# minfenli/refnerf-pl

Hardware: AMD Instinct MI355X
Metric: ray-samples/s (4096 rays x 128 samples x 2 levels, Ref-NeRF Blender, eval forward) (higher is better)
Workload: dtype f16x2; 1 GPU; blender_refnerf.gin, 4096 rays x 128 samples, 2-level, Model.__call__ eval forward with compute_extras + full ray_history; rays_per_gpu=4096, total_rays=4096, samples_per_level=128, parallelism=ray-tile dp1, n_ranks_seen=1, hip_graph_replay=False

## Files before the change

### refnerf-pl_amd/csrc/refnerf_level_bf16.h

```cpp
#pragma once
#include <type_traits>

#include "refnerf_level_common.h"

namespace rn {

typedef short v2s __attribute__((ext_vector_type(2)));

struct MmBf16 {
  typedef __bf16 t;
  typedef t v8 __attribute__((ext_vector_type(8)));
  typedef t v2 __attribute__((ext_vector_type(2)));
  static __device__ __forceinline__ v16f mfma(v8 a, v8 b, v16f c) { return __builtin_amdgcn_mfma_f32_32x32x16_bf16(a, b, c, 0, 0, 0); }
};
struct MmF16 {
  typedef _Float16 t;
  typedef t v8 __attribute__((ext_vector_type(8)));
  typedef t v2 __attribute__((ext_vector_type(2)));
  static __device__ __forceinline__ v16f mfma(v8 a, v8 b, v16f c) { return __builtin_amdgcn_mfma_f32_32x32x16_f16(a, b, c, 0, 0, 0); }
};
template <typename MM>
__device__ __forceinline__ unsigned cvt_pk_mm(float lo, float hi) {
  typename MM::v2 r = __builtin_convertvector((v2f){lo, hi}, typename MM::v2);
  return __builtin_bit_cast(unsigned, r);
// ... 428 lines not shown
  if (KIND == SQ_BN) return 2 * (j / 4) + (j & 1);
  if (KIND == SQ_SC) return 2 * (j / 3) + ((j % 3) == 1 ? 1 : 0);
  return 4 * (j / 6) + ((j % 6) < 4 ? (j % 6) : (j % 6) - 4);
}
template <int KIND> constexpr bool sq_lo(int j) { return KIND == SQ_BN ? (j & 3) >= 2 : (KIND == SQ_SC ? (j % 3) == 2 : (j % 6) >= 4); }
template <int KIND> constexpr int sq_tile(int j) { return KIND == SQ_SC ? 0 : (KIND == SQ_BN ? (j & 1) : ((j % 6) & 1)); }
template <int KIND> constexpr int sq_release(int j) {
  if (KIND == SQ_BN) return (j & 3) >= 2 ? 2 * (j / 4) + ((j & 3) - 2) : -1;
  if (KIND == SQ_SC) return (j % 3) == 1 ? 2 * (j / 3) + 1 : ((j % 3) == 2 ? 2 * (j / 3) : -1);
  const int jj = j % 6, sl = j / 6;
  return jj == 2 ? 4 * sl + 2 : (jj == 3 ? 4 * sl + 3 : (jj == 4 ? 4 * sl : (jj == 5 ? 4 * sl + 1 : -1)));
}
template <int KIND, bool PRE, typename Hook = NoHook>
__device__ __forceinline__ void sq_chunk(Pipe &p, sq_v8 (&fr)[SQ_NF], const v4uu (&in)[16], SqAcc &acc, SqAcc &nacc, Hook &&hook = Hook(), int adv = BF_CHUNK_BYTES) {
  constexpr int NM = sq_nm<KIND>(), NP = sq_np<KIND>();
  constexpr int RDV = NM / 2 - 1;
  const char *w = p.wbuf + p.cur_off;
  const char *cur = w + 1024 + p.lane * 16;
  const char *nxt = p.wbuf + p.nxt_off + 1024 + p.lane * 16;
  sq_v8 xb[2];
  if (KIND == SQ_X) { xb[0] = lds_frag<MmF16>(p.xps); xb[1] = lds_frag<MmF16>(p.xps + (BT / 2) * 16); }
  __builtin_amdgcn_sched_barrier(0);
#pragma unroll
  for (int j = 0; j < NM; ++j) {
    const int sl = sq_step<KIND>(j);
    sq_v8 b;
    if (KIND == SQ_X) b = xb[sq_lo<KIND>(j) ? 1 : 0];
    else b = __builtin_bit_cast(sq_v8, in[2 * ((KIND == SQ_B ? 4 : 0) + sl) + (sq_lo<KIND>(j) ? 1 : 0)]);
    if (sq_tile<KIND>(j)) acc.t1 = __builtin_amdgcn_mfma_f32_16x16x32_f16(fr[sq_piece<KIND>(j) % SQ_NF], b, acc.t1, 0, 0, 0);
    else acc.t0 = __builtin_amdgcn_mfma_f32_16x16x32_f16(fr[sq_piece<KIND>(j) % SQ_NF], b, acc.t0, 0, 0, 0);
    const int rel = sq_release<KIND>(j);
    if (rel >= 0) {
      const int q = rel + SQ_NF;
      fr[rel % SQ_NF] = (q < NP) ? lds_frag<MmF16>(cur + q * 1024) : lds_frag<MmF16>(nxt + (q - NP) * 1024);
    }
    hook(j);
    if (KIND == SQ_X) {
      if ((j % 6) == 3 && sl + 1 < 3) xb[0] = lds_frag<MmF16>(p.xps + (sl + 1) * (4 * BT * 16));
      if ((j % 6) == 5 && sl + 1 < 3) xb[1] = lds_frag<MmF16>(p.xps + (sl + 1) * (4 * BT * 16) + (BT / 2) * 16);
    }
    if (j == RDV) {
      RN_RENDEZVOUS(p);
      issue_chunk<true>(p, p.fil_off, 0);
      if (PRE) {
        const v4f *bp = reinterpret_cast<const v4f *>(p.wbuf + p.nxt_off + (p.lane >> 4) * 16);
        nacc.t0 = bp[0];
        nacc.t1 = bp[4];
      }
    }
    if (j == RDV + 4) issue_chunk<true>(p, p.fil_off, 1);
    if (j == RDV + 8) issue_chunk<true>(p, p.fil_off, 2, adv);
    __builtin_amdgcn_sched_barrier(0);
  }
  ring_rotate(p);
}
__device__ __forceinline__ void sq_epi_piece(const SqAcc &a, int q, v4uu &oh, v4uu &ol) {
  const float y0 = q == 0 ? a.t0[0] : (q == 1 ? a.t0[2] : (q == 2 ? a.t1[0] : a.t1[2]));
  const float y1 = q == 0 ? a.t0[1] : (q == 1 ? a.t0[3] : (q == 2 ? a.t1[1] : a.t1[3]));
  const float x0 = (y0 < 0.0f) ? 0.0f : y0, x1 = (y1 < 0.0f) ? 0.0f : y1;
  unsigned hi, lo;
  split_pair_f16(x0, x1, hi, lo);
  oh[q] = hi;
  ol[q] = lo;
}
template <bool LAYER0>
__device__ __forceinline__ void sq_layer(Pipe &p, sq_v8 (&fr)[SQ_NF], SqAcc (&accs)[2], bool skip, const v4uu (&in)[16], v4uu (&out)[16]) {
#pragma unroll
  for (int ob = 0; ob < 8; ++ob) {
    SqAcc &acc = accs[(ob + 1) & 1];
    SqAcc &prev = accs[ob & 1];
    auto hook = [&](int j) {
      if (ob == 0 || j >= 8 || (j & 1)) return;
      sq_epi_piece(prev, j >> 1, out[2 * ob - 2], out[2 * ob - 1]);
    };
    if constexpr (LAYER0) sq_chunk<SQ_XR, true>(p, fr, in, acc, prev, hook);
    else {
      sq_chunk<SQ_A, false>(p, fr, in, acc, prev, hook);
      sq_chunk<SQ_B, true>(p, fr, in, acc, prev);
      if (skip) sq_chunk<SQ_X, true>(p, fr, in, acc, prev);
    }
  }
#pragma unroll
  for (int q = 0; q < 4; ++q) sq_epi_piece(accs[0], q, out[14], out[15]);
  __builtin_amdgcn_sched_barrier(0);
}
__device__ __forceinline__ void sq_load_ipe_frags(const Pipe &p, v4uu (&in)[16]) {
#pragma unroll
  for (int s = 0; s < 3; ++s) {
    in[2 * s] = __builtin_bit_cast(v4uu, lds_frag<MmF16>(p.xps + s * (4 * BT * 16)));
    in[2 * s + 1] = __builtin_bit_cast(v4uu, lds_frag<MmF16>(p.xps + s * (4 * BT * 16) + (BT / 2) * 16));
  }
}
__device__ __forceinline__ void sq_bias_now(const Pipe &p, SqAcc &acc) {
  const v4f *bp = reinterpret_cast<const v4f *>(p.wbuf + p.cur_off + (p.lane >> 4) * 16);
  acc.t0 = bp[0];
  acc.t1 = bp[4];
}

template <typename MM, int KIND0, int REAL0>
__device__ __forceinline__ void dir_layer(Pipe &p, typename MM::v8 (&a)[AF], int second, const v4uu (&in)[16], const v4uu (&bn)[8], v4uu (&out)[16], int adv6 = BF_CHUNK_BYTES) {
#pragma unroll
  for (int ob = 0; ob < 8; ++ob) {
    v16f acc;
    bf_chunk<MM, KIND0, REAL0, true, true>(p, a, in, bn, acc, NoHook(), ob == 6 ? adv6 : BF_CHUNK_BYTES);
    if constexpr (KIND0 == BF_REG) {
      if (second == 2) bf_chunk<MM, BF_BNLDS, BF_DIR_REAL_KS, false, true>(p, a, in, bn, acc);
    }
    pack_acc<MM, true>(acc, out[2 * ob], out[2 * ob + 1]);
    __builtin_amdgcn_sched_barrier(0);
  }
}

template <bool RINGPS = false>
__device__ __forceinline__ void level_fwd_split(const LevelArgs &A) {
  typedef MmF16 MM;
  constexpr int PSM = RINGPS ? BF_PS_RING - 1 : 0;
  typedef typename MM::v8 v8mm;
  typedef typename MM::t mm_t;
  extern __shared__ __attribute__((aligned(16))) float smem[];
  const refnerf_level_cfg &cfg = A.cfg;
  const int N = cfg.n_samples;
  const int tid = threadIdx.x, lane = tid & 63;
  const int wave = __builtin_amdgcn_readfirstlane(tid >> 6);
  const int rpw = A.rpw;
  const int ray0 = blockIdx.x * rpw;
  const int n_tot = rpw * N;
  const int n_pass = (n_tot + BT - 1) / BT;

  char *WB = reinterpret_cast<char *>(smem);
  char *Xb = WB + BF_RING_BYTES;
  float *HD = reinterpret_cast<float *>(Xb + BF_X_BYTES);
  float *TD = HD + HD_ROWS * BT;
  float *XP = TD + rpw * (N + 1);
  float *PS = XP + rpw * (N + 1);
  float *PX = PS + (RINGPS ? BF_PS_RING : n_tot) * NPS_EVAL;
  float *NRM = PX + 3 * BT;
  const float *RY = NRM + 8;

  const int h = lane >> 5, n = lane & 31;
  const int col = wave * 32 + n;

  Pipe p;
  pipe_stream_init(p, A.packed, n_pass * SPPACKED.chunks_per_pass, wave, lane);
  p.wbuf = WB;
  p.xp = Xb + (h * BT + col) * 16;
  p.xps = Xb + ((lane >> 4) * BT + wave * 16 + (lane & 15)) * 16;
  p.cur_off = 0; p.nxt_off = BF_CHUNK_BYTES; p.fil_off = 2 * BF_CHUNK_BYTES;
  p.lane = lane; p.wave = wave; p.h = h;
  p.t_vm = 0; p.t_bar = 0;
  RN_STAMPW(A, 0);
#ifdef REFNERF_PROF_WAITS
  if (A.prof && blockIdx.x == (gridDim.x >> 1) && lane == 0) A.prof[wave * 32 + 22] = (long long)__builtin_amdgcn_s_memrealtime();
#endif
  issue_chunk<true>(p, p.cur_off);
  issue_chunk<true>(p, p.nxt_off);

  resample_phase<BF_NW, true>(A, reinterpret_cast<float *>(Xb), TD, NRM, ray0, wave, lane);
#pragma clang loop unroll(disable)
  for (int rl = wave; rl < rpw; rl += BF_NW) {
    const int ray = ray0 + rl;
    if (ray >= A.R) break;
    float *RYw = NRM + 8 + rl * 12;
    if (lane < 10) {
      const float val = lane < 3 ? A.rays.d_origins[(size_t)ray * 3 + lane]
                      : lane < 6 ? A.rays.d_directions[(size_t)ray * 3 + lane - 3]
                      : lane < 9 ? A.rays.d_viewdirs[(size_t)ray * 3 + lane - 6] : A.rays.d_radii[ray];
      RYw[lane] = val;
      const float dx = __shfl(val, 3, 64), dy = __shfl(val, 4, 64), dz = __shfl(val, 5, 64);
      if (lane == 0) NRM[rl] = sqrtf((dx * dx + dy * dy) + dz * dz);
    }
  }
  RN_STAMPW(A, 1);
  asm volatile("s_waitcnt vmcnt(0)" ::: "memory");
  __syncthreads();
  RN_STAMPW(A, 2);

  if (wave >= BF_NW / 2) __builtin_amdgcn_s_setprio(1);
  v4uu R0[16], R1[16];
  sq_v8 ar[SQ_NF];
#pragma unroll
  for (int d = 0; d < SQ_NF; ++d) ar[d] = lds_frag<MM>(WB + 1024 + lane * 16 + d * 1024);

  for (int pass0 = 0; pass0 < n_tot; pass0 += BT) {
    int lane_v = lane;
    asm volatile("" : "+v"(lane_v));
    p.lane_off = (unsigned)(wave * 3072 + lane_v * 16);
    auto locate = [&](int &g, int &rl, bool &valid) {
      int col_l = col, pass_l = pass0;
      asm volatile("" : "+v"(col_l), "+s"(pass_l));
      g = pass_l + col_l;
      rl = g / N;
      valid = (g < n_tot) && (ray0 + rl < A.R);
    };
    auto pass_epilogue = [&]() {
      if constexpr (RINGPS) {
        __syncthreads();
        const int end = (pass0 + BT < n_tot) ? pass0 + BT : n_tot;
        int td_o = (int)(TD - smem), xp_o = (int)(XP - smem), ps_o = (int)(PS - smem), nrm_o = (int)(NRM - smem), lane_e = lane, pass_e = pass0;
        int ntot_e = n_tot, ray0_e = ray0, wave_e = wave;
        asm volatile("" : "+s"(td_o), "+s"(xp_o), "+s"(ps_o), "+s"(nrm_o), "+v"(lane_e), "+s"(pass_e), "+s"(ntot_e), "+s"(ray0_e), "+s"(wave_e));
        composite_phase<BF_NW, false, NPS_EVAL, PSM>(A, smem + td_o, smem + xp_o, smem + ps_o, ntot_e, ray0_e, wave_e, lane_e, nullptr, smem + nrm_o,
                                                     pass_e / N, end / N);
      }
    };
    {
      const int g0 = pass0 + wave * 32;
      if (g0 >= n_tot || ray0 + g0 / N >= A.R) { idle_pass<true>(p); pass_epilogue(); continue; }
    }
    auto load_heads = [&](SampleHeads &sh, int &g, bool &valid) {
      int rl;
      locate(g, rl, valid);
      int ci = col, ro = (valid ? rl : 0) * 12;
      asm volatile("" : "+v"(ci), "+v"(ro));
      float v[3], gp[3], raw_dif[3], raw_tint[3];
#pragma unroll
      for (int i = 0; i < 3; ++i) {
        v[i] = RY[ro + 6 + i];
        gp[i] = HD[(1 + i) * BT + ci];
        raw_dif[i] = HD[(5 + i) * BT + ci];
        raw_tint[i] = HD[(8 + i) * BT + ci];
      }
      sample_heads<false>(cfg, HD[0 * BT + ci], gp, HD[4 * BT + ci], raw_dif, raw_tint, v, sh);
    };

    v4uu bn0[4];
    auto heads = [&](auto RUN, v4uu (&bn)[8]) {
      constexpr int run = decltype(RUN)::value;
      SqAcc ha[2];
      sq_bias_now(p, ha[1]);
#pragma unroll
      for (int ob = 0; ob < 5; ++ob) {
        SqAcc &acc = ha[(ob + 1) & 1];
        if (ob < 4) {
          sq_chunk<SQ_BN, true>(p, ar, R1, acc, ha[ob & 1], NoHook(), (run == 0 && ob == 2) ? SP_ADV_REWIND : BF_CHUNK_BYTES);
#pragma unroll
          for (int e = 0; e < 4; ++e) {
            const unsigned pk = e == 0 ? pk_f16(acc.t0[0], acc.t0[1]) : (e == 1 ? pk_f16(acc.t0[2], acc.t0[3])
                              : (e == 2 ? pk_f16(acc.t1[0], acc.t1[1]) : pk_f16(acc.t1[2], acc.t1[3])));
            if (run == 0) bn0[ob][e] = pk;
            else {
              const v2uu r = __builtin_amdgcn_permlane16_swap(bn0[ob][e], pk, false, false);
              bn[2 * ob][e] = r[0];
              bn[2 * ob + 1][e] = r[1];
            }
          }
        } else {
          sq_chunk<SQ_SC, false>(p, ar, R1, acc, ha[ob & 1]);
          const int bq = lane_v >> 4;
          int csl = wave * 32 + 16 * run + (lane_v & 15) + 4 * bq * BT;
          asm volatile("" : "+v"(csl));
#pragma unroll
          for (int i = 0; i < 4; ++i)
            if (4 * bq + i < HD_ROWS) HD[i * BT + csl] = acc.t0[i];
        }
      }
      wave_sync();
    };
    typedef std::integral_constant<int, 0> Run0;
    typedef std::integral_constant<int, 1> Run1;

#pragma unroll 1
    for (int phase = 0; phase < 2; ++phase) {
#pragma unroll
      for (int e = 0; e < 16; ++e) { R0[e] = (v4uu){0, 0, 0, 0}; R1[e] = (v4uu){0, 0, 0, 0}; }
      {
      const int i16 = lane_v & 15, part = lane_v >> 4;
      const int hb = part >> 1, qq = part & 1;
      const int cs = wave * 32 + 16 * phase + i16;
      const int gs = pass0 + cs;
      const int rls = gs / N, sis = gs - rls * N;
      const bool vs = (gs < n_tot) && (ray0 + rls < A.R);
      float o[3], d[3];
      const float *ry = RY + (vs ? rls : 0) * 12;
#pragma unroll
      for (int i = 0; i < 3; ++i) { o[i] = ry[i]; d[i] = ry[3 + i]; }
      const float radius = ry[9];
      const float *td = TD + (vs ? rls : 0) * (N + 1);
      const float t0 = td[vs ? sis : 0], t1 = td[vs ? sis + 1 : 1];
      float lm[3], lv[3];
      cast_sample(o, d, radius, t0, t1, cfg.ray_shape, lm, lv);
      if (cfg.disable_integration) { lv[0] = 0.0f; lv[1] = 0.0f; lv[2] = 0.0f; }
      char *xw = Xb + (wave * 16 + i16) * 16;
      RN_STAMPW(A, 17);
      float sc = qq ? 256.0f : 1.0f, sc2 = qq ? 65536.0f : 1.0f;
      char *xq = xw + (6 * hb + 3 * qq) * BT * 16;
#pragma clang loop unroll(disable)
      for (int dp = 0; dp < 4; ++dp) {
        const float sc_odd = sc * 2.0f, sc2_odd = sc2 * 4.0f;
#pragma unroll
        for (int a = 0; a < 3; ++a) {
          float f[2];
#pragma unroll
          for (int u = 0; u < 2; ++u) {
            const int k6 = 2 * a + u, odd = k6 / 3, b3 = k6 - 3 * odd;
            f[u] = ipe_feature_split_sc(lm[b3], lv[b3], odd ? sc_odd : sc, odd ? sc2_odd : sc2, hb);
          }
          unsigned whi, wlo;
          split_pair_f16(f[0], f[1], whi, wlo);
          const int t = 3 * dp + a;
          char *dst = xq + (t >> 2) * BT * 16 + (t & 3) * 4;
          *reinterpret_cast<unsigned *>(dst) = whi;
          *reinterpret_cast<unsigned *>(dst + (BT / 2) * 16) = wlo;
        }
        sc *= 4.0f;
        sc2 *= 16.0f;
      }
      }
      RN_STAMPW(A, 18);
      wave_sync();
      RN_STAMPW(A, 3 + phase * 4);
      if (phase == 0) {
#pragma unroll
        for (int d = AF; d < SQ_NF; ++d) ar[d] = lds_frag<MM>(p.wbuf + p.cur_off + 1024 + lane_v * 16 + d * 1024);
      }
      SqAcc accs[2];
      sq_bias_now(p, accs[1]);
      sq_load_ipe_frags(p, R1);
      sq_layer<true>(p, ar, accs, false, R1, R0);
#pragma unroll
      for (int e = 0; e < 6; ++e) R1[e] = (v4uu){0, 0, 0, 0};
      RN_STAMPW(A, 4 + phase * 4);
#pragma unroll 1
      for (int it = 0; it < 4; ++it) {
        sq_layer<false>(p, ar, accs, it == 2, R0, R1);
        if (it < 3) sq_layer<false>(p, ar, accs, false, R1, R0);
      }
      RN_STAMPW(A, 5 + phase * 4);
      if (phase == 0) {
        v4uu none[8];
        heads(Run0(), none);
        RN_STAMPW(A, 6);
      }
    }
    v4uu bn[8];
    heads(Run1(), bn);
    RN_STAMPW(A, 10);
#pragma unroll
    for (int e = 0; e < 16; ++e) { R0[e] = (v4uu){0, 0, 0, 0}; R1[e] = (v4uu){0, 0, 0, 0}; }
    {
    const int h4 = RINGPS ? (fresh_lane() >> 5) : h;
    char *xs = Xb + col * 16;
    {
      SampleHeads sh;
      int g4; bool valid4;
      load_heads(sh, g4, valid4);
      if (valid4 && h4 == 0) heads_store<NPS_EVAL, PSM>(sh, PS, PX, g4, RINGPS ? wave * 32 + (fresh_lane() & 31) : col);
      float ide[40];
#pragma unroll
      for (int q = 36; q < 40; ++q) ide[q] = 0.0f;
      if (cfg.dir_enc == REFNERF_DIRENC_POSENC) posenc_eval<false, true>(sh.refd[0], sh.refd[1], sh.refd[2], h4, [&](int q, float val) { ide[q] = val; });
      else ide_eval<false>(sh.refd[0], sh.refd[1], sh.refd[2], sh.rough, h4, [&](int q, float val) { ide[q] = val; });
      if (h4 == 0) ide[36] = sh.dot;
#pragma unroll
      for (int q = 0; q < 5; ++q) {
        v8mm pk;
#pragma unroll
        for (int e = 0; e < 8; ++e) pk[e] = (mm_t)ide[q * 8 + e];
        *reinterpret_cast<v8mm *>(xs + (5 * h4 + q) * BT * 16) = pk;
      }
    }
    wave_sync();
    RN_STAMPW(A, 11);
    v8mm (&ad)[AF] = reinterpret_cast<v8mm (&)[AF]>(ar);
    dir_layer<MM, BF_BNLDS, BF_DIR_REAL_KS>(p, ad, 0, R0, bn, R0);
    RN_STAMPW(A, 12);
#pragma unroll 1
    for (int it = 0; it < 4; ++it) {
      dir_layer<MM, BF_REG, 0>(p, ad, (it == 2) ? 2 : 0, R0, bn, R1, it == 3 ? SP_ADV_WRAP : BF_CHUNK_BYTES);
      if (it < 3) dir_layer<MM, BF_REG, 0>(p, ad, 0, R1, bn, R0);
    }
    RN_STAMPW(A, 13);
    v16f acc;
    bf_chunk<MM, BF_REG, 0, true, true>(p, ad, R1, bn, acc);
    float raw_rgb[3];
    const int lane6 = RINGPS ? fresh_lane() : lane;
    const int n6 = RINGPS ? (lane6 & 31) : n, h6 = RINGPS ? (lane6 >> 5) : h;
#pragma unroll
    for (int i = 0; i < 3; ++i) raw_rgb[i] = __shfl(acc[i], n6, 64);
    int g_w, rl_w; bool valid;
    locate(g_w, rl_w, valid);
    int lane_w = lane6, pass_w = pass0;
    asm volatile("" : "+v"(lane_w), "+s"(pass_w));
    if (valid) {
      int ci = RINGPS ? wave * 32 + n6 : col, pr = ps_row<PSM>(g_w) * NPS_EVAL;
      asm volatile("" : "+v"(ci), "+v"(pr));
      float tint[3], raw_dif[3];
#pragma unroll
      for (int i = 0; i < 3; ++i) { tint[i] = PS[pr + PS_TINT + i]; raw_dif[i] = HD[(5 + i) * BT + ci]; }
      int half = h6;
      asm volatile("" : "+v"(half));
      colour_store_halves<NPS_EVAL, PSM, true>(A, half, tint, raw_dif, raw_rgb, PS, g_w);
    }
    wave_sync();
    history_flush<NPS_EVAL, PSM>(A, PS, PX, n_tot, pass_w + wave * 32, wave * 32, (size_t)ray0 * N + pass_w + wave * 32, lane_w);
    RN_STAMPW(A, 14);
    }
    __builtin_amdgcn_wave_barrier();
    pass_epilogue();
  }
  asm volatile("s_waitcnt vmcnt(0)" ::: "memory");
  __syncthreads();
  RN_STAMPW(A, 15);
#ifdef REFNERF_PROF_WAITS
  if (A.prof && blockIdx.x == (gridDim.x >> 1) && lane == 0) {
    A.prof[wave * 32 + 20] = p.t_vm; A.prof[wave * 32 + 21] = p.t_bar;
    A.prof[wave * 32 + 23] = (long long)__builtin_amdgcn_s_memrealtime();
  }
#endif
  if constexpr (!RINGPS) composite_phase<BF_NW, false, NPS_EVAL>(A, TD, XP, PS, n_tot, ray0, wave, lane, reinterpret_cast<float *>(WB), NRM);
  RN_STAMPW(A, 16);
}

#ifndef REFNERF_SECONDARY_TU
__global__ __launch_bounds__(BF_NTHREADS) void level_fwd_f16x2(const LevelArgs A) { level_fwd_split<false>(A); }
__global__ __launch_bounds__(BF_NTHREADS) void level_fwd_f16x2_ring(const LevelArgs A) { level_fwd_split<true>(A); }
#endif

__device__ __forceinline__ int ipe_col_of_kprime(int kp) { return kp; }

}
```

### refnerf-pl_amd/csrc/refnerf_level_common.h

```cpp
#pragma once
#include <hip/hip_runtime.h>

#include "refnerf_hip.h"
#include "refnerf_device_math.h"
#include "refnerf_layout.h"

namespace rn {

typedef float v16f __attribute__((ext_vector_type(16)));
typedef float v4f __attribute__((ext_vector_type(4)));
typedef unsigned int v4u __attribute__((ext_vector_type(4)));

constexpr int NTHREADS = 256;

typedef __bf16 v8bf __attribute__((ext_vector_type(8)));
typedef unsigned v4uu __attribute__((ext_vector_type(4)));
typedef __bf16 v2bf __attribute__((ext_vector_type(2)));
typedef float v2f __attribute__((ext_vector_type(2)));
__device__ __forceinline__ unsigned cvt_pk_bf16(float lo, float hi) {
  v2bf r = __builtin_convertvector((v2f){lo, hi}, v2bf);
  return __builtin_bit_cast(unsigned, r);
}

constexpr int HD_ROWS = 12;
// ... 43 lines not shown
#pragma unroll
  for (int o = 32; o > 0; o >>= 1) v += __shfl_xor(v, o, 64);
  return v;
}
__device__ __forceinline__ float wave_max(float v) {
#pragma unroll
  for (int o = 32; o > 0; o >>= 1) v = fmaxf(v, __shfl_xor(v, o, 64));
  return v;
}
constexpr int WSUM_PITCH = 65;
template <int K>
__device__ __forceinline__ void wave_sum_many(float (&v)[K], float *scr, int lane) {
#pragma unroll
  for (int k = 0; k < K; ++k) scr[k * WSUM_PITCH + lane] = v[k];
  __builtin_amdgcn_fence(__ATOMIC_SEQ_CST, "wavefront");
  __builtin_amdgcn_wave_barrier();
  float s = 0.0f;
  if (lane < K) {
    const float *col = scr + lane * WSUM_PITCH;
#pragma clang loop unroll(disable)
    for (int j = 0; j < 64; j += 4) s += (col[j] + col[j + 1]) + (col[j + 2] + col[j + 3]);
  }
#pragma unroll
  for (int k = 0; k < K; ++k) v[k] = __shfl(s, k, 64);
  __builtin_amdgcn_fence(__ATOMIC_SEQ_CST, "wavefront");
  __builtin_amdgcn_wave_barrier();
}

__device__ __forceinline__ float lane_value(float x, int l) {
  return __builtin_bit_cast(float, __builtin_amdgcn_readlane(__builtin_bit_cast(int, x), l));
}

__device__ __forceinline__ double wave_scan_incl(double v, int lane) {
#pragma unroll
  for (int o = 1; o < 64; o <<= 1) {
    double t = __shfl_up(v, o, 64);
    if (lane >= o) v += t;
  }
  return v;
}

__device__ __forceinline__ float cdf_interp(float u, float xp0, float xp1, float fp0, float fp1) {
  float q = (u - xp0) / (xp1 - xp0);
  if (q != q) q = 0.0f;
  float off = clip01(q);
  return fp0 + off * (fp1 - fp0);
}

__device__ __forceinline__ void centres_to_sdist(const float *c, int N, float smin, float smax, float *sd, int lane) {
  __builtin_amdgcn_fence(__ATOMIC_SEQ_CST, "wavefront");
  __builtin_amdgcn_wave_barrier();
  #pragma clang loop unroll(disable)
  for (int k = lane; k <= N; k += 64) {
    float v;
    if (k == 0) v = fmaxf(smin, 2.0f * c[0] - (c[1] + c[0]) / 2.0f);
    else if (k == N) v = fminf(smax, 2.0f * c[N - 1] - (c[N - 1] + c[N - 2]) / 2.0f);
    else v = (c[k] + c[k - 1]) / 2.0f;
    sd[k] = v;
  }
  __builtin_amdgcn_fence(__ATOMIC_SEQ_CST, "wavefront");
  __builtin_amdgcn_wave_barrier();
}

template <bool EXACT = true>
__device__ __forceinline__ void build_cdf_wave(float *lg, float *cw, int M, int lane) {
  float mx = -INFINITY;
  #pragma clang loop unroll(disable)
  for (int i = lane; i < M; i += 64) mx = fmaxf(mx, lg[i]);
  mx = wave_max(mx);
  #pragma clang loop unroll(disable)
  for (int i = lane; i < M; i += 64) lg[i] = rn_det_expf(lg[i] - mx);
  __builtin_amdgcn_fence(__ATOMIC_SEQ_CST, "wavefront");
  __builtin_amdgcn_wave_barrier();
  float sum = 0.0f;
  if (EXACT) {
    #pragma clang loop unroll(disable)
    for (int i0 = 0; i0 < M; i0 += 64) {
      const float x = (i0 + lane < M) ? lg[i0 + lane] : 0.0f;
#pragma unroll
      for (int l = 0; l < 64; ++l) sum += lane_value(x, l);
    }
  } else {
    #pragma clang loop unroll(disable)
    for (int i = lane; i < M; i += 64) sum += lg[i];
    sum = wave_sum(sum);
  }
  #pragma clang loop unroll(disable)
  for (int i = lane; i < M; i += 64) lg[i] = lg[i] / sum;
  __builtin_amdgcn_fence(__ATOMIC_SEQ_CST, "wavefront");
  __builtin_amdgcn_wave_barrier();
  if (EXACT) {
    double acc = 0.0;
    #pragma clang loop unroll(disable)
    for (int i0 = 0; i0 < M; i0 += 64) {
      const float x = (i0 + lane < M) ? lg[i0 + lane] : 0.0f;
      float mine = 0.0f;
#pragma unroll
      for (int l = 0; l < 64; ++l) {
        acc += (double)lane_value(x, l);
        mine = (lane == l) ? (float)acc : mine;
      }
      if (i0 + lane < M - 1) cw[i0 + lane + 1] = fminf(1.0f, mine);
    }
    if (lane == 0) { cw[0] = 0.0f; cw[M] = 1.0f; }
  } else {
    const int Cn = (M + 63) / 64, i0 = lane * Cn;
    double loc = 0.0;
    #pragma clang loop unroll(disable)
    for (int q = 0; q < Cn; ++q) if (i0 + q < M - 1) loc += (double)lg[i0 + q];
    double run = wave_scan_incl(loc, lane) - loc;
    #pragma clang loop unroll(disable)
    for (int q = 0; q < Cn; ++q) if (i0 + q < M - 1) { run += (double)lg[i0 + q]; cw[i0 + q + 1] = fminf(1.0f, (float)run); }
    if (lane == 0) { cw[0] = 0.0f; cw[M] = 1.0f; }
  }
  __builtin_amdgcn_fence(__ATOMIC_SEQ_CST, "wavefront");
  __builtin_amdgcn_wave_barrier();
}

__device__ __forceinline__ void invert_cdf_wave(const float *t_in, const float *cw, float *c, int M, int N, float smin, float smax,
                                                float *sd, int32_t *bin_idx_g, int lane) {
  #pragma clang loop unroll(disable)
  for (int k = lane; k < N; k += 64) {
    float u = linspace_u(k, N);
    int lo = 0, hi = M;
    #pragma clang loop unroll(disable)
    while (hi - lo > 1) {
      int mid = (lo + hi) >> 1;
      if (u >= cw[mid]) lo = mid; else hi = mid;
    }
    c[k] = cdf_interp(u, cw[lo], cw[lo + 1], t_in[lo], t_in[lo + 1]);
    if (bin_idx_g) bin_idx_g[k] = lo;
  }
  centres_to_sdist(c, N, smin, smax, sd, lane);
}

template <bool EXACT = true>
__device__ __forceinline__ void sample_intervals_wave(const float *t_in, float *lg, float *cw, float *c, int M, int N,
                                      float smin, float smax, float *sd, int32_t *bin_idx_g, int lane) {
  build_cdf_wave<EXACT>(lg, cw, M, lane);
  invert_cdf_wave(t_in, cw, c, M, N, smin, smax, sd, bin_idx_g, lane);
}

__device__ __forceinline__ int fresh_lane() {
  int z = 0;
  asm volatile("" : "+v"(z));
  return (int)__builtin_amdgcn_mbcnt_hi(~0u, __builtin_amdgcn_mbcnt_lo(~0u, (unsigned)z));
}

__device__ __forceinline__ void st3(float *base, size_t idx, float a, float b, float c) {
  if (base) { base[idx * 3 + 0] = a; base[idx * 3 + 1] = b; base[idx * 3 + 2] = c; }
}


template <int NW = 4, bool EXACT = true>
__device__ __forceinline__ void resample_phase(const LevelArgs &A, float *scratch, float *TD, float *NRM, int ray0, int wave, int lane) {
  const refnerf_level_cfg &cfg = A.cfg;
  const int N = cfg.n_samples, M = cfg.n_in, rpw = A.rpw;
  const int Mp = (M + 4) & ~3, Np = (N + 3) & ~3;
  float *scr = scratch + wave * (3 * Mp + Np);
  float *t_in = scr, *lg = scr + Mp, *cw = scr + 2 * Mp, *c = scr + 3 * Mp;
  #pragma clang loop unroll(disable)
  for (int rl = wave; rl < rpw; rl += NW) {
    int ray = ray0 + rl;
    if (ray >= A.R) break;
    float *sd = TD + rl * (N + 1);
    int32_t *bin_g = A.out.d_bin_idx ? A.out.d_bin_idx + (size_t)ray * N : nullptr;
    if (A.sdist_in == nullptr) {
      t_in[0] = cfg.s_near; t_in[1] = cfg.s_far;
      cw[0] = 0.0f; cw[1] = 1.0f;
      wave_sync();
    } else {
      const float *tg = A.sdist_in + (size_t)ray * (M + 1);
      const float *wg = A.weights_in + (size_t)ray * M;
      #pragma clang loop unroll(disable)
      for (int i = lane; i <= M; i += 64) t_in[i] = tg[i];
      wave_sync();
      RN_STAMP_P0(A, 24);
      #pragma clang loop unroll(disable)
      for (int i = lane; i < M; i += 64)
        lg[i] = (t_in[i + 1] > t_in[i]) ? cfg.anneal * rn_det_logf(wg[i] + cfg.resample_padding) : -INFINITY;
      wave_sync();
      RN_STAMP_P0(A, 25);
      build_cdf_wave<EXACT>(lg, cw, M, lane);
    }
    RN_STAMP_P0(A, 26);
    invert_cdf_wave(t_in, cw, c, M, N, cfg.s_near, cfg.s_far, sd, bin_g, lane);
    RN_STAMP_P0(A, 27);
    float nearv = A.rays.d_near[ray], farv = A.rays.d_far[ray];
    if (!EXACT) {
      float *RY = NRM + 8 + rl * 12;
      if (lane < 10) {
        const float val = lane < 3 ? A.rays.d_origins[(size_t)ray * 3 + lane]
                        : lane < 6 ? A.rays.d_directions[(size_t)ray * 3 + lane - 3]
                        : lane < 9 ? A.rays.d_viewdirs[(size_t)ray * 3 + lane - 6] : A.rays.d_radii[ray];
        RY[lane] = val;
        const float dx = __shfl(val, 3, 64), dy = __shfl(val, 4, 64), dz = __shfl(val, 5, 64);
        if (lane == 0) NRM[rl] = sqrtf((dx * dx + dy * dy) + dz * dz);
      }
    }
    RN_STAMP_P0(A, 28);
    #pragma clang loop unroll(disable)
    for (int k = lane; k <= N; k += 64) {
      float s = sd[k];
      if (A.out.d_sdist) A.out.d_sdist[(size_t)ray * (N + 1) + k] = s;
      sd[k] = s_to_t(s, nearv, farv, A.cfg.raydist);
    }
  }
}

struct SampleHeads {
  float density, rough, dot;
  float tint[3], raw_dif[3], npred[3], gp[3], refd[3];
  float normals[3] = {0.0f, 0.0f, 0.0f};
};
template <bool FAST = false>
__device__ __forceinline__ void sample_heads(const refnerf_level_cfg &cfg, float raw_density, const float gp[3],
                                             float raw_rough, const float raw_dif[3], const float raw_tint[3],
                                             const float v[3], SampleHeads &s) {
#pragma unroll
  for (int i = 0; i < 3; ++i) { s.gp[i] = gp[i]; s.raw_dif[i] = raw_dif[i]; s.tint[i] = sigmoid_m<FAST>(raw_tint[i]); }
  float n2 = fmaxf((gp[0] * gp[0] + gp[1] * gp[1]) + gp[2] * gp[2], EPS32);
  float nrm = sqrtf(n2);
#pragma unroll
  for (int i = 0; i < 3; ++i) s.npred[i] = -m_div<FAST>(gp[i], nrm);
  s.density = softplus_m<FAST>(raw_density + cfg.density_bias);
  s.rough = softplus_m<FAST>(raw_rough + cfg.roughness_bias);
  float w3[3] = {-v[0], -v[1], -v[2]};
  float dot = (s.npred[0] * w3[0] + s.npred[1] * w3[1]) + s.npred[2] * w3[2];
#pragma unroll
  for (int i = 0; i < 3; ++i) s.refd[i] = (2.0f * dot) * s.npred[i] - w3[i];
  s.dot = (s.npred[0] * v[0] + s.npred[1] * v[1]) + s.npred[2] * v[2];
}

template <int PSM>
__device__ __forceinline__ int ps_row(int g) { return PSM ? (g & PSM) : g; }

template <bool FAST = false, int NP = NPS_TRAIN, int PSM = 0, bool FAST_SRGB = FAST, bool PAD_HERE = false>
__device__ __forceinline__ void colour_store(const LevelArgs &A, const SampleHeads &s, const float raw_rgb[3],
                                             float *PS, float *PX, int n_tot, int g_sample, int gcol) {
  const int g = ps_row<PSM>(g_sample);
  const refnerf_level_cfg &cfg = A.cfg;
  float spec_lin[3], dif_lin[3], rgb[3], dif[3], spc[3];
#pragma unroll
  for (int i = 0; i < 3; ++i) {
    float sg = sigmoid_m<FAST>(cfg.rgb_premultiplier * raw_rgb[i] + cfg.rgb_bias);
    dif_lin[i] = sigmoid_m<FAST>(s.raw_dif[i] - LOG3_F);
    spec_lin[i] = s.tint[i] * sg;
    rgb[i] = spec_lin[i] + dif_lin[i];
  }
  if (cfg.srgb_mapping) {
    if (cfg.srgb_mapping_normalization) {
      float norm = fmaxf(fmaxf(fmaxf(rgb[0], rgb[1]), rgb[2]), 1.0f);
#pragma unroll
      for (int i = 0; i < 3; ++i) rgb[i] = m_div<FAST>(rgb[i], norm);
    }
#pragma unroll
    for (int i = 0; i < 3; ++i) {
      rgb[i] = clip01(linear_to_srgb<FAST_SRGB>(rgb[i]));
      dif[i] = clip01(linear_to_srgb<FAST_SRGB>(dif_lin[i]));
      spc[i] = clip01(linear_to_srgb<FAST_SRGB>(spec_lin[i]));
    }
  } else {
#pragma unroll
    for (int i = 0; i < 3; ++i) { dif[i] = dif_lin[i]; spc[i] = spec_lin[i]; }
  }
  float pad = cfg.rgb_padding;
  if (PAD_HERE) asm volatile("" : "+s"(pad));
  const float pad_scale = (float)(1.0 + 2.0 * (double)pad);
#pragma unroll
  for (int i = 0; i < 3; ++i) rgb[i] = rgb[i] * pad_scale - pad;
  PS[g * NP + PS_DENSITY] = s.density;
  PS[g * NP + PS_ROUGH] = s.rough;
#pragma unroll
  for (int i = 0; i < 3; ++i) {
    PS[g * NP + PS_RGB + i] = rgb[i];
    PS[g * NP + PS_DIF + i] = dif[i];
    PS[g * NP + PS_SPC + i] = spc[i];
    PS[g * NP + PS_NPRED + i] = s.npred[i];
    PS[g * NP + PS_TINT + i] = s.tint[i];
    if (NP > PS_NORMALS) PS[g * NP + PS_NORMALS + i] = s.normals[i];
    PX[gcol * 3 + i] = s.gp[i];
  }
}

template <int NP, int PSM>
__device__ __forceinline__ void heads_store(const SampleHeads &s, float *PS, float *PX, int g_sample, int gcol) {
  const int g = ps_row<PSM>(g_sample);
  PS[g * NP + PS_DENSITY] = s.density;
  PS[g * NP + PS_ROUGH] = s.rough;
#pragma unroll
  for (int i = 0; i < 3; ++i) {
    PS[g * NP + PS_NPRED + i] = s.npred[i];
    PS[g * NP + PS_TINT + i] = s.tint[i];
    PX[gcol * 3 + i] = s.gp[i];
  }
}
template <int NP, int PSM, bool PAD_HERE>
__device__ __forceinline__ void colour_store_halves(const LevelArgs &A, int half, const float tint[3], const float raw_dif[3],
                                                    const float raw_rgb[3], float *PS, int g_sample) {
  const int g = ps_row<PSM>(g_sample);
  const refnerf_level_cfg &cfg = A.cfg;
  float own[3], rgb[3];
#pragma unroll
  for (int i = 0; i < 3; ++i) {
    const float sg = sigmoid_m<false>(half ? raw_dif[i] - LOG3_F : cfg.rgb_premultiplier * raw_rgb[i] + cfg.rgb_bias);
    own[i] = half ? sg : tint[i] * sg;
  }
#pragma unroll
  for (int i = 0; i < 3; ++i) rgb[i] = own[i] + __shfl_xor(own[i], 32, 64);
  if (cfg.srgb_mapping) {
    if (cfg.srgb_mapping_normalization) {
      float norm = fmaxf(fmaxf(fmaxf(rgb[0], rgb[1]), rgb[2]), 1.0f);
#pragma unroll
      for (int i = 0; i < 3; ++i) rgb[i] = m_div<false>(rgb[i], norm);
    }
#pragma unroll
    for (int i = 0; i < 3; ++i) {
      rgb[i] = clip01(linear_to_srgb<true>(rgb[i]));
      own[i] = clip01(linear_to_srgb<true>(own[i]));
    }
  }
  float pad = cfg.rgb_padding;
  if (PAD_HERE) asm volatile("" : "+s"(pad));
  const float pad_scale = (float)(1.0 + 2.0 * (double)pad);
  const int own_slot = half ? PS_DIF : PS_SPC;
#pragma unroll
  for (int i = 0; i < 3; ++i) {
    PS[g * NP + own_slot + i] = own[i];
    if (!half) PS[g * NP + PS_RGB + i] = rgb[i] * pad_scale - pad;
  }
}

__device__ __forceinline__ void hist_store(float *p, float v) { __builtin_nontemporal_store(v, p); }
constexpr int AUX_NT = 2;

template <int NP = NPS_TRAIN, int PSM = 0>
__device__ __forceinline__ void history_flush(const LevelArgs &A, const float *PS, const float *PX, int n_tot, int gw0, int gcol0,
                                              size_t gs0, int lane) {
  const size_t total = (size_t)A.R * A.cfg.n_samples;
  auto vec3 = [&](float *dst, int slot) {
    if (!dst) return;
#pragma unroll
    for (int it = 0; it < 2; ++it) {
      const int f = lane + 64 * it;
      const int smp = f / 3, c = f - 3 * smp;
      if (f < 96 && gw0 + smp < n_tot && gs0 + smp < total) hist_store(dst + gs0 * 3 + f, PS[ps_row<PSM>(gw0 + smp) * NP + slot + c]);
    }
  };
  auto scal = [&](float *dst, int slot) {
    if (dst && lane < 32 && gw0 + lane < n_tot && gs0 + lane < total) hist_store(dst + gs0 + lane, PS[ps_row<PSM>(gw0 + lane) * NP + slot]);
  };
  scal(A.out.d_density, PS_DENSITY);
  scal(A.out.d_roughness, PS_ROUGH);
  vec3(A.out.d_rgb, PS_RGB);
  vec3(A.out.d_diffuse, PS_DIF);
  vec3(A.out.d_specular, PS_SPC);
  vec3(A.out.d_normals_pred, PS_NPRED);
  if (A.out.d_grad_pred) {
#pragma unroll
    for (int it = 0; it < 2; ++it) {
      const int f = lane + 64 * it;
      const int smp = f / 3;
      if (f < 96 && gw0 + smp < n_tot && gs0 + smp < total) hist_store(A.out.d_grad_pred + gs0 * 3 + f, PX[gcol0 * 3 + f]);
    }
  }
  vec3(A.out.d_tint, PS_TINT);
  if (NP > PS_NORMALS && A.cfg.training) vec3(A.out.d_normals, PS_NORMALS);
}

template <typename T>
__device__ __forceinline__ T *late_ptr(T *p) {
  asm volatile("" : "+s"(p));
  return p;
}

__device__ __forceinline__ void pct_store(double *soa, double *aos, int R, int ray, int p, double v) {
  if (soa) soa[(size_t)p * R + ray] = v;
  else aos[(size_t)ray * 3 + p] = v;
}

template <int NW = 4, bool FAST = false, int NP = NPS_TRAIN, int PSM = 0>
__device__ __forceinline__ void composite_phase(const LevelArgs &A, const float *TD, float *XP, float *PS, int n_tot,
                                                int ray0, int wave, int lane, float *wscr, const float *NRM,
                                                int rl_begin = 0, int rl_end = -1) {
  const refnerf_level_cfg &cfg = A.cfg;
  const int N = cfg.n_samples, rpw = A.rpw;
  if (rl_end < 0) rl_end = rpw;
  #pragma clang loop unroll(disable)
  for (int rl = rl_begin + wave; rl < rl_end; rl += NW) {
    const int ray = ray0 + rl;
    if (ray >= A.R) break;
    const float *td = TD + rl * (N + 1);
    const int base = rl * N;
    const int C = (N + 63) / 64;
    const int i0 = lane * C;
    float norm;
    if (FAST) norm = NRM[rl];
    else {
      float dx = A.rays.d_directions[(size_t)ray * 3], dy = A.rays.d_directions[(size_t)ray * 3 + 1], dz = A.rays.d_directions[(size_t)ray * 3 + 2];
      norm = sqrtf((dx * dx + dy * dy) + dz * dz);
    }
    auto wref = [&](int i) -> float & { return PS[ps_row<PSM>(base + i) * NP + PS_DENSITY]; };
    auto rec = [&](int i, int slot) { return PS[ps_row<PSM>(base + i) * NP + slot]; };
    double local = 0.0;
    #pragma clang loop unroll(disable)
    for (int q = 0; q < C; ++q) {
      int i = i0 + q;
      if (i < N) {
        float dd = wref(i) * ((td[i + 1] - td[i]) * norm);
        if (!(cfg.opaque_background && i == N - 1)) local += (double)dd;
      }
    }
    double incl = wave_scan_incl(local, lane);
    double cum = incl - local;
    float acc = 0, s_rgb[3] = {0, 0, 0}, s_dif[3] = {0, 0, 0}, s_spc[3] = {0, 0, 0}, s_np[3] = {0, 0, 0}, s_tn[3] = {0, 0, 0};
    float s_nm[3] = {0, 0, 0};
    float s_dist = 0, s_rgh = 0, s_logd = 0;
    double wlocal = 0.0;
    #pragma clang loop unroll(disable)
    for (int q = 0; q < C; ++q) {
      int i = i0 + q;
      if (i < N) {
        float dd = wref(i) * ((td[i + 1] - td[i]) * norm);
        if (cfg.opaque_background && i == N - 1) dd = INFINITY;
        float alpha = 1.0f - m_exp<FAST>(-dd);
        float trans = m_exp<FAST>(-(float)cum);
        float w = alpha * trans;
        cum += (double)dd;
        wref(i) = w;
        wlocal += (double)w;
        if (A.out.d_weights) A.out.d_weights[(size_t)ray * N + i] = w;
        acc += w;
        float tmid = 0.5f * (td[i] + td[i + 1]);
        s_dist += w * tmid;
        s_logd += w * m_log<FAST>(tmid);
        s_rgh += w * rec(i, PS_ROUGH);
#pragma unroll
        for (int c = 0; c < 3; ++c) {
          s_rgb[c] += w * rec(i, PS_RGB + c);
          s_dif[c] += w * rec(i, PS_DIF + c);
          s_spc[c] += w * rec(i, PS_SPC + c);
          s_np[c] += w * rec(i, PS_NPRED + c);
          s_tn[c] += w * rec(i, PS_TINT + c);
          if (NP > PS_NORMALS) s_nm[c] += w * rec(i, PS_NORMALS + c);
        }
      }
    }
    {
      float red[22] = {acc, s_dist, s_logd, s_rgh, s_rgb[0], s_rgb[1], s_rgb[2], s_dif[0], s_dif[1], s_dif[2],
                       s_spc[0], s_spc[1], s_spc[2], s_np[0], s_np[1], s_np[2], s_tn[0], s_tn[1], s_tn[2],
                       s_nm[0], s_nm[1], s_nm[2]};
      if constexpr (PSM != 0) {
#pragma unroll
        for (int k = 0; k < 22; ++k) red[k] = wave_sum(red[k]);
      } else wave_sum_many<22>(red, wscr + wave * (22 * WSUM_PITCH), lane);
      acc = red[0]; s_dist = red[1]; s_logd = red[2]; s_rgh = red[3];
#pragma unroll
      for (int c = 0; c < 3; ++c) {
        s_rgb[c] = red[4 + c]; s_dif[c] = red[7 + c]; s_spc[c] = red[10 + c];
        s_np[c] = red[13 + c]; s_tn[c] = red[16 + c]; s_nm[c] = red[19 + c];
      }
    }
    const float bg_w = fmaxf(0.0f, 1.0f - acc);
    float rgb[3], dif[3], spc[3];
#pragma unroll
    for (int c = 0; c < 3; ++c) {
      rgb[c] = s_rgb[c] + bg_w * cfg.bg_rgb; dif[c] = s_dif[c] + bg_w * cfg.bg_rgb; spc[c] = s_spc[c] + bg_w * cfg.bg_rgb;
    }
    const int mode = cfg.render_srgb_mode;
    if (mode != REFNERF_SRGB_NONE) {
      if (mode == REFNERF_SRGB_NORM_LINEAR || mode == REFNERF_SRGB_NORM_SRGB) {
        float nr = fmaxf(fmaxf(fmaxf(rgb[0], rgb[1]), rgb[2]), 1.0f);
#pragma unroll
        for (int c = 0; c < 3; ++c) rgb[c] = rgb[c] / nr;
      }
#pragma unroll
      for (int c = 0; c < 3; ++c) {
        if (mode == REFNERF_SRGB_SRGB || mode == REFNERF_SRGB_NORM_SRGB) {
          rgb[c] = linear_to_srgb<FAST>(rgb[c]); dif[c] = linear_to_srgb<FAST>(dif[c]); spc[c] = linear_to_srgb<FAST>(spc[c]);
        }
        rgb[c] = clip01(rgb[c]); dif[c] = clip01(dif[c]); spc[c] = clip01(spc[c]);
      }
    }
    if (lane == 0) {
      st3(A.out.d_r_rgb, ray, rgb[0], rgb[1], rgb[2]);
      st3(late_ptr(A.xout.d_r_rgb_fg), ray, s_rgb[0], s_rgb[1], s_rgb[2]);
      st3(A.out.d_r_diffuse, ray, dif[0], dif[1], dif[2]);
      st3(A.out.d_r_specular, ray, spc[0], spc[1], spc[2]);
      if (A.out.d_r_distance) A.out.d_r_distance[ray] = s_dist;
      if (A.out.d_r_acc) A.out.d_r_acc[ray] = acc;
      if (cfg.compute_extras) {
        if (cfg.training) {
          if (NP > PS_NORMALS) st3(A.out.d_r_normals, ray, s_nm[0], s_nm[1], s_nm[2]);
          else {
            float z = 0.0f;
            asm volatile("" : "+v"(z));
            st3(A.out.d_r_normals, ray, z, z, z);
          }
        }
        st3(A.out.d_r_normals_pred, ray, s_np[0], s_np[1], s_np[2]);
        st3(A.out.d_r_tint, ray, s_tn[0], s_tn[1], s_tn[2]);
        if (A.out.d_r_roughness) A.out.d_r_roughness[ray] = s_rgh;
        if (A.out.d_r_distance_mean) {
          float e = expf(s_logd / fmaxf(EPS32, acc));
          if (e != e) e = INFINITY;
          e = fminf(fmaxf(e, td[0]), td[N]);
          A.out.d_r_distance_mean[ray] = e;
        }
      }
    }
    double *const pct_soa = late_ptr(A.xout.d_r_percentiles_soa), *const pct_aos = A.out.d_r_percentiles;
    if (cfg.compute_extras && (pct_aos || pct_soa)) {
      float *xp = XP + rl * (N + 1);
      double wincl = wave_scan_incl(wlocal, lane);
      double run = wincl - wlocal;
      __builtin_amdgcn_wave_barrier();
      #pragma clang loop unroll(disable)
      for (int q = 0; q < C; ++q) {
        int i = i0 + q;
        if (i < N) { run += (double)wref(i); xp[i + 1] = fminf(1.0f, (float)run); }
      }
      if (lane == 0) { xp[0] = 0.0f; }
      __builtin_amdgcn_fence(__ATOMIC_SEQ_CST, "wavefront");
      __builtin_amdgcn_wave_barrier();
      const float farv = A.rays.d_far[ray];
      const double psd[3] = {(double)(5.0f / 100.0f), (double)(50.0f / 100.0f), (double)(95.0f / 100.0f)};
      const int nk = N + 2;
      if (FAST) {
        int cnt[3] = {0, 0, 0};
        #pragma clang loop unroll(disable)
        for (int j0 = 0; j0 < nk; j0 += 64) {
          const int j = j0 + lane;
          const bool in = j < nk;
          const double xj = (!in || j == nk - 1) ? 1.0 : (double)xp[j];
#pragma unroll
          for (int p = 0; p < 3; ++p) cnt[p] += __builtin_popcountll(__builtin_amdgcn_ballot_w64(in && psd[p] >= xj));
        }
        if (lane < 3) {
          const double x = lane == 0 ? psd[0] : (lane == 1 ? psd[1] : psd[2]);
          int idx = (lane == 0 ? cnt[0] : (lane == 1 ? cnt[1] : cnt[2])) - 1;
          if (idx < 0) idx = 0;
          if (idx > nk - 2) idx = nk - 2;
          double x0 = (double)xp[idx], x1 = (idx + 1 == nk - 1) ? 1.0 : (double)xp[idx + 1];
          double f0 = (double)td[idx], f1 = (idx + 1 == nk - 1) ? (double)farv : (double)td[idx + 1];
          double m = (f1 - f0) / (x1 - x0);
          double b = f0 - m * x0;
          pct_store(pct_soa, pct_aos, A.R, ray, lane, m * x + b);
        }
      } else {
        #pragma clang loop unroll(disable)
        for (int p = 0; p < 3; ++p) {
          double x = psd[p];
          int cnt = 0;
          #pragma clang loop unroll(disable)
          for (int j = lane; j < nk; j += 64) {
            double xj = (j == nk - 1) ? 1.0 : (double)xp[j];
            cnt += (x >= xj) ? 1 : 0;
          }
#pragma unroll
          for (int o2 = 32; o2 > 0; o2 >>= 1) cnt += __shfl_xor(cnt, o2, 64);
          if (lane == 0) {
            int idx = cnt - 1;
            if (idx < 0) idx = 0;
            if (idx > nk - 2) idx = nk - 2;
            double x0 = (double)xp[idx], x1 = (idx + 1 == nk - 1) ? 1.0 : (double)xp[idx + 1];
            double f0 = (double)td[idx], f1 = (idx + 1 == nk - 1) ? (double)farv : (double)td[idx + 1];
            double m = (f1 - f0) / (x1 - x0);
            double b = f0 - m * x0;
            pct_store(pct_soa, pct_aos, A.R, ray, p, m * x + b);
          }
        }
      }
    }
  }
}

}
```

Baseline: 279.1 million ray-samples/s.

## Prefetch ray attributes and first-ray knots into LDS before resampling

Adds a prologue that loads per-ray origins, directions, viewdirs, radii, near and far into the LDS ray record, and loads the first ray's input knots and weights with four loads in flight per lane. The prologue runs before the weight-stream chunks are issued. The resample and composite phases then read near, far and the direction norm from LDS instead of global memory, and composite switches to the fast ballot-based percentile path. The aim is to cut dependent global-load latency at kernel start and inside composite. The cost is a larger ray record and an extra wave_sync before the weight stream is issued, and the percentile change may differ slightly numerically.

Result: no change. 279.3 million ray-samples/s (median of 6 runs) (+0.1%).

```diff
diff --git a/refnerf-pl_amd/csrc/refnerf_level_bf16.h b/refnerf-pl_amd/csrc/refnerf_level_bf16.h
--- a/refnerf-pl_amd/csrc/refnerf_level_bf16.h
+++ b/refnerf-pl_amd/csrc/refnerf_level_bf16.h
@@ -604,24 +604,11 @@
 #ifdef REFNERF_PROF_WAITS
   if (A.prof && blockIdx.x == (gridDim.x >> 1) && lane == 0) A.prof[wave * 32 + 22] = (long long)__builtin_amdgcn_s_memrealtime();
 #endif
+  resample_prologue<BF_NW>(A, reinterpret_cast<float *>(Xb), NRM, ray0, wave, lane);
   issue_chunk<true>(p, p.cur_off);
   issue_chunk<true>(p, p.nxt_off);
 
-  resample_phase<BF_NW, true>(A, reinterpret_cast<float *>(Xb), TD, NRM, ray0, wave, lane);
-#pragma clang loop unroll(disable)
-  for (int rl = wave; rl < rpw; rl += BF_NW) {
-    const int ray = ray0 + rl;
-    if (ray >= A.R) break;
-    float *RYw = NRM + 8 + rl * 12;
-    if (lane < 10) {
-      const float val = lane < 3 ? A.rays.d_origins[(size_t)ray * 3 + lane]
-                      : lane < 6 ? A.rays.d_directions[(size_t)ray * 3 + lane - 3]
-                      : lane < 9 ? A.rays.d_viewdirs[(size_t)ray * 3 + lane - 6] : A.rays.d_radii[ray];
-      RYw[lane] = val;
-      const float dx = __shfl(val, 3, 64), dy = __shfl(val, 4, 64), dz = __shfl(val, 5, 64);
-      if (lane == 0) NRM[rl] = sqrtf((dx * dx + dy * dy) + dz * dz);
-    }
-  }
+  resample_phase<BF_NW, true, true>(A, reinterpret_cast<float *>(Xb), TD, NRM, ray0, wave, lane);
   RN_STAMPW(A, 1);
   asm volatile("s_waitcnt vmcnt(0)" ::: "memory");
   __syncthreads();
@@ -651,7 +638,7 @@
         int td_o = (int)(TD - smem), xp_o = (int)(XP - smem), ps_o = (int)(PS - smem), nrm_o = (int)(NRM - smem), lane_e = lane, pass_e = pass0;
         int ntot_e = n_tot, ray0_e = ray0, wave_e = wave;
         asm volatile("" : "+s"(td_o), "+s"(xp_o), "+s"(ps_o), "+s"(nrm_o), "+v"(lane_e), "+s"(pass_e), "+s"(ntot_e), "+s"(ray0_e), "+s"(wave_e));
-        composite_phase<BF_NW, false, NPS_EVAL, PSM>(A, smem + td_o, smem + xp_o, smem + ps_o, ntot_e, ray0_e, wave_e, lane_e, nullptr, smem + nrm_o,
+        composite_phase<BF_NW, false, NPS_EVAL, PSM, true>(A, smem + td_o, smem + xp_o, smem + ps_o, ntot_e, ray0_e, wave_e, lane_e, nullptr, smem + nrm_o,
                                                      pass_e / N, end / N);
       }
     };
@@ -859,7 +846,7 @@
     A.prof[wave * 32 + 23] = (long long)__builtin_amdgcn_s_memrealtime();
   }
 #endif
-  if constexpr (!RINGPS) composite_phase<BF_NW, false, NPS_EVAL>(A, TD, XP, PS, n_tot, ray0, wave, lane, reinterpret_cast<float *>(WB), NRM);
+  if constexpr (!RINGPS) composite_phase<BF_NW, false, NPS_EVAL, 0, true>(A, TD, XP, PS, n_tot, ray0, wave, lane, reinterpret_cast<float *>(WB), NRM);
   RN_STAMPW(A, 16);
 }
 
diff --git a/refnerf-pl_amd/csrc/refnerf_level_common.h b/refnerf-pl_amd/csrc/refnerf_level_common.h
--- a/refnerf-pl_amd/csrc/refnerf_level_common.h
+++ b/refnerf-pl_amd/csrc/refnerf_level_common.h
@@ -219,7 +219,7 @@
 }
 
 
-template <int NW = 4, bool EXACT = true>
+template <int NW = 4, bool EXACT = true, bool PARKED = false>
 __device__ __forceinline__ void resample_phase(const LevelArgs &A, float *scratch, float *TD, float *NRM, int ray0, int wave, int lane) {
   const refnerf_level_cfg &cfg = A.cfg;
   const int N = cfg.n_samples, M = cfg.n_in, rpw = A.rpw;
@@ -232,6 +232,7 @@
     if (ray >= A.R) break;
     float *sd = TD + rl * (N + 1);
     int32_t *bin_g = A.out.d_bin_idx ? A.out.d_bin_idx + (size_t)ray * N : nullptr;
+    const bool have_knots = PARKED && rl == wave;
     if (A.sdist_in == nullptr) {
       t_in[0] = cfg.s_near; t_in[1] = cfg.s_far;
       cw[0] = 0.0f; cw[1] = 1.0f;
@@ -239,13 +240,21 @@
     } else {
       const float *tg = A.sdist_in + (size_t)ray * (M + 1);
       const float *wg = A.weights_in + (size_t)ray * M;
-      #pragma clang loop unroll(disable)
-      for (int i = lane; i <= M; i += 64) t_in[i] = tg[i];
+      if (!have_knots) {
+        #pragma clang loop unroll(disable)
+        for (int i = lane; i <= M; i += 64) t_in[i] = tg[i];
+      }
       wave_sync();
       RN_STAMP_P0(A, 24);
-      #pragma clang loop unroll(disable)
-      for (int i = lane; i < M; i += 64)
-        lg[i] = (t_in[i + 1] > t_in[i]) ? cfg.anneal * rn_det_logf(wg[i] + cfg.resample_padding) : -INFINITY;
+      if (have_knots) {
+        #pragma clang loop unroll(disable)
+        for (int i = lane; i < M; i += 64)
+          lg[i] = (t_in[i + 1] > t_in[i]) ? cfg.anneal * rn_det_logf(lg[i] + cfg.resample_padding) : -INFINITY;
+      } else {
+        #pragma clang loop unroll(disable)
+        for (int i = lane; i < M; i += 64)
+          lg[i] = (t_in[i + 1] > t_in[i]) ? cfg.anneal * rn_det_logf(wg[i] + cfg.resample_padding) : -INFINITY;
+      }
       wave_sync();
       RN_STAMP_P0(A, 25);
       build_cdf_wave<EXACT>(lg, cw, M, lane);
@@ -253,7 +262,9 @@
     RN_STAMP_P0(A, 26);
     invert_cdf_wave(t_in, cw, c, M, N, cfg.s_near, cfg.s_far, sd, bin_g, lane);
     RN_STAMP_P0(A, 27);
-    float nearv = A.rays.d_near[ray], farv = A.rays.d_far[ray];
+    float nearv, farv;
+    if (PARKED) { const float *RYp = NRM + 8 + rl * 12; nearv = RYp[10]; farv = RYp[11]; }
+    else { nearv = A.rays.d_near[ray]; farv = A.rays.d_far[ray]; }
     if (!EXACT) {
       float *RY = NRM + 8 + rl * 12;
       if (lane < 10) {
@@ -270,9 +281,54 @@
     for (int k = lane; k <= N; k += 64) {
       float s = sd[k];
       if (A.out.d_sdist) A.out.d_sdist[(size_t)ray * (N + 1) + k] = s;
-      sd[k] = s_to_t(s, nearv, farv, A.cfg.raydist);
-    }
-  }
+      float nv = nearv, fv = farv;
+      if (PARKED) asm volatile("" : "+v"(nv), "+v"(fv));
+      sd[k] = s_to_t(s, nv, fv, A.cfg.raydist);
+    }
+  }
+}
+
+template <int NW>
+__device__ __forceinline__ void resample_prologue(const LevelArgs &A, float *scratch, float *NRM, int ray0, int wave, int lane) {
+  const int N = A.cfg.n_samples, M = A.cfg.n_in, rpw = A.rpw;
+  const int Mp = (M + 4) & ~3, Np = (N + 3) & ~3;
+  float *scr = scratch + wave * (3 * Mp + Np);
+  float *t_in = scr, *lg = scr + Mp;
+  #pragma clang loop unroll(disable)
+  for (int rl = wave; rl < rpw; rl += NW) {
+    const int ray = ray0 + rl;
+    if (ray >= A.R) break;
+    const float *src = lane < 3 ? A.rays.d_origins + ((size_t)ray * 3 + lane)
+                     : lane < 6 ? A.rays.d_directions + ((size_t)ray * 3 + lane - 3)
+                     : lane < 9 ? A.rays.d_viewdirs + ((size_t)ray * 3 + lane - 6)
+                     : lane == 9 ? A.rays.d_radii + ray : lane == 10 ? A.rays.d_near + ray : A.rays.d_far + ray;
+    const float val = lane < 12 ? *src : 0.0f;
+    if (rl == wave && A.sdist_in != nullptr) {
+      const float *tg = A.sdist_in + (size_t)ray * (M + 1);
+      const float *wg = A.weights_in + (size_t)ray * M;
+      #pragma clang loop unroll(disable)
+      for (int b = lane; b <= M; b += 256) {
+        float tv[4], wv[4];
+#pragma unroll
+        for (int u = 0; u < 4; ++u) {
+          const int i = b + 64 * u;
+          tv[u] = i <= M ? tg[i] : 0.0f;
+          wv[u] = i < M ? wg[i] : 0.0f;
+        }
+#pragma unroll
+        for (int u = 0; u < 4; ++u) {
+          const int i = b + 64 * u;
+          if (i <= M) t_in[i] = tv[u];
+          if (i < M) lg[i] = wv[u];
+        }
+      }
+    }
+    float *RYw = NRM + 8 + rl * 12;
+    if (lane < 12) RYw[lane] = val;
+    const float dx = __shfl(val, 3, 64), dy = __shfl(val, 4, 64), dz = __shfl(val, 5, 64);
+    if (lane == 0) NRM[rl] = sqrtf((dx * dx + dy * dy) + dz * dz);
+  }
+  wave_sync();
 }
 
 struct SampleHeads {
@@ -446,7 +502,7 @@
   else aos[(size_t)ray * 3 + p] = v;
 }
 
-template <int NW = 4, bool FAST = false, int NP = NPS_TRAIN, int PSM = 0>
+template <int NW = 4, bool FAST = false, int NP = NPS_TRAIN, int PSM = 0, bool PARKED = false>
 __device__ __forceinline__ void composite_phase(const LevelArgs &A, const float *TD, float *XP, float *PS, int n_tot,
                                                 int ray0, int wave, int lane, float *wscr, const float *NRM,
                                                 int rl_begin = 0, int rl_end = -1) {
@@ -462,7 +518,7 @@
     const int C = (N + 63) / 64;
     const int i0 = lane * C;
     float norm;
-    if (FAST) norm = NRM[rl];
+    if (FAST || PARKED) norm = NRM[rl];
     else {
       float dx = A.rays.d_directions[(size_t)ray * 3], dy = A.rays.d_directions[(size_t)ray * 3 + 1], dz = A.rays.d_directions[(size_t)ray * 3 + 2];
       norm = sqrtf((dx * dx + dy * dy) + dz * dz);
@@ -590,10 +646,10 @@
       if (lane == 0) { xp[0] = 0.0f; }
       __builtin_amdgcn_fence(__ATOMIC_SEQ_CST, "wavefront");
       __builtin_amdgcn_wave_barrier();
-      const float farv = A.rays.d_far[ray];
+      const float farv = PARKED ? NRM[8 + rl * 12 + 11] : A.rays.d_far[ray];
       const double psd[3] = {(double)(5.0f / 100.0f), (double)(50.0f / 100.0f), (double)(95.0f / 100.0f)};
       const int nk = N + 2;
-      if (FAST) {
+      if (FAST || PARKED) {
         int cnt[3] = {0, 0, 0};
         #pragma clang loop unroll(disable)
         for (int j0 = 0; j0 < nk; j0 += 64) {
```
